# myshell-ai/OpenVoice

Measured on NVIDIA H100. Metric: audio_seconds_per_second, higher is better.
Workload: dtype f32 (3xFP16 split-precision tensor-core convs with fp32 accumulation, fp32 FFMA elsewhere)

## Files before the change

openvoice_b200/csrc/ovc_lib.cu:

```cuda
#include <cuda_runtime.h>

#include <algorithm>
#include <cmath>
#include <cstdarg>
#include <cstdio>
#include <cstdlib>
#include <cstring>
#include <map>
#include <string>
#include <vector>

#include "../../include/ovc.h"
#include "ovc_convpack.h"
#include "ovc_small.cuh"
#include "ovc_tcconv.cuh"
#include "ovc_tts.cuh"
#include "ovc_refenc.cuh"
#include "ovc_resample.cuh"
#include "ovc_splice.h"
#include "ovc_variants.h"

namespace ovc {

static thread_local std::string g_err;
// ... 98 lines not shown
  int n_vocab = 0, n_speakers = 0, H = 0, C = 0, Fc = 0, heads = 0, n_layers = 0, window = 0, D = 0;
  size_t emb = 0, emb_g = 0;
  std::vector<TcLayer> qkv, o;
  std::vector<Fp32Dense> ffn1, ffn2;
  std::vector<size_t> relk, relv, ln1g, ln1b, ln2g, ln2b;
  TcLayer proj;
  Fp32Dense dp_c1, dp_c2, sdp_pre, sdp_proj;
  size_t dp_n1g = 0, dp_n1b = 0, dp_n2g = 0, dp_n2b = 0, dp_pw = 0, dp_pb = 0, dp_cw = 0, dp_cb = 0, sdp_cw = 0, sdp_cb = 0,
         ea = 0;
  DdsLayers dds[4];
  size_t cf_pre_w[4] = {0}, cf_pre_b[4] = {0}, cf_pw[4] = {0}, cf_pb[4] = {0};
};

struct DebugBuf {
  float* d = nullptr;
  int64_t shape[4] = {0, 0, 0, 0};
  size_t floats = 0;
};

}

using namespace ovc;

struct ovc_ctx {
  ovc_hparams hp{};
  int device = 0;
  int sm_count = 0;
  std::map<std::string, HostTensor> sd;
  bool finalized = false;

  float* d_w = nullptr;
  size_t w_floats = 0;
  std::vector<float> h_w;

  ConvLayer enc_pre, enc_pre16, enc_proj;
  WNLayers enc_wn;
  ConvLayer flow_pre[4], flow_post[4];
  WNLayers flow_wn[4];
  ConvLayer dec_pre, dec_ups[4];
  ConvLayer rb_c1[12][3], rb_c2[12][3];
  TcLayer tc_c1[12][3], tc_c2[12][3], tc_ups[4], tc_pre;
  float* d_tcw = nullptr;
  std::vector<float> h_tcw;
  int precision = 0;
  bool tts_simple = false;
  bool use_graph = true;
  int use_pdl = 2;
  bool use_branches = true;
  int par_frames = 512;
  bool use_pair = true;
  bool use_pair_occ = true;
  bool use_staged_epi = true;
  bool pair_occ2_ok[TCN_N_OCC2] = {};
  cudaStream_t br_stream[2] = {nullptr, nullptr};
  cudaEvent_t br_ev[4] = {nullptr, nullptr, nullptr, nullptr};
  size_t post_w_off = 0;
  size_t cond_w_off = 0, cond_b_off = 0;
  int* d_cond_wrow = nullptr;
  int* d_cond_sel = nullptr;
  int cond_rows_out = 0;
  int cond_off_enc = 0, cond_off_fsrc = 0, cond_off_ftgt = 0, cond_off_dec = 0;
  int cond_off_enc_tc = 0, cond_off_fsrc_tc = 0, cond_off_ftgt_tc = 0;
  int* d_cond_cols[2][3] = {};
  int cond_pf_cols[2][3] = {};
  int cond_pf_off[2][3][4] = {};

  float2* d_tw = nullptr;
  float* d_win = nullptr;

  bool has_refenc = false;
  size_t re_conv_w[6] = {0}, re_conv_b[6] = {0}, re_wih = 0, re_whh = 0, re_bih = 0, re_bhh = 0, re_pw = 0, re_pb = 0,
         re_lng = 0, re_lnb = 0;
  int re_gru_in = 0;
  float* d_re = nullptr;
  size_t re_floats = 0;
  float* d_res = nullptr;
  size_t res_floats = 0;

  std::map<std::pair<int64_t, int64_t>, double*> rs_banks;
  bool rs_smem_opt_in = false;
  std::vector<RsRingPlan> rs_plans;
  RsRingPlan* d_rs_plans = nullptr;
  int rs_ring_tile = 256;
  size_t rs_ring_smem = 0;

  float* d_ws = nullptr;
  size_t ws_floats = 0;

  TtsLayers tts;
  float* d_tts = nullptr;
  size_t tts_floats = 0;
  int tts_B = 0, tts_T = 0;
  bool tts_gtok = false;

  bool prof = false;
  std::vector<cudaEvent_t> ev;
  size_t ev_used = 0;
  double prof_ms = 0, prof_flops = 0, prof_bytes = 0;
  int64_t prof_launches = 0;
  std::vector<double> ev_flops, ev_bytes;
  std::vector<int> ev_variant, ev_family, ev_tag;

  bool debug = false;
  std::map<std::string, DebugBuf> taps;

  int launches = 0;
// ... 348 lines not shown
      auto col = [&](int i) { return cols.empty() ? i : cols[i]; };
      for (int i = 0; i < n; ++i)
        if (sel[col(i)] != sel[col(i / COND_ROWS * COND_ROWS)]) return false;
      return true;
    };
    bool ok = uniform({}, (int)sel.size());
    for (auto& oc : pf_cols)
      for (auto& cols : oc) ok = ok && uniform(cols, (int)cols.size());
    if (!ok) return fail(OVC_ERR_INVALID, "conditioning sections are not aligned to %d rows", COND_ROWS);
  }
  c->has_refenc = false;
  if (find(c, "ref_enc.proj.weight")) {
    static const int filt[7] = {1, 32, 32, 64, 64, 128, 128};
    for (int i = 0; i < 6; ++i) {
      const std::string q = "ref_enc.convs." + std::to_string(i);
      HostTensor w;
      const HostTensor* b;
      TRY(conv_weight(c, q, {filt[i + 1], filt[i], 3, 3}, &w));
      TRY(tensor(c, q + ".bias", {filt[i + 1]}, &b));
      c->re_conv_w[i] = append(c->h_w, w.data);
      c->re_conv_b[i] = append(c->h_w, b->data);
    }
    int w6 = S;
    for (int i = 0; i < 6; ++i) w6 = (w6 - 1) / 2 + 1;
    c->re_gru_in = 128 * w6;
    const struct { const char* key; std::vector<int64_t> shape; size_t* off; } re[8] = {
        {"ref_enc.gru.weight_ih_l0", {384, c->re_gru_in}, &c->re_wih}, {"ref_enc.gru.weight_hh_l0", {384, 128}, &c->re_whh},
        {"ref_enc.gru.bias_ih_l0", {384}, &c->re_bih},                 {"ref_enc.gru.bias_hh_l0", {384}, &c->re_bhh},
        {"ref_enc.proj.weight", {G, 128}, &c->re_pw},                  {"ref_enc.proj.bias", {G}, &c->re_pb},
        {"ref_enc.layernorm.weight", {S}, &c->re_lng},                 {"ref_enc.layernorm.bias", {S}, &c->re_lnb}};
    for (const auto& e : re) {
      const HostTensor* t;
      TRY(tensor(c, e.key, e.shape, &t));
      *e.off = append(c->h_w, t->data);
    }
    c->has_refenc = true;
  }
  c->tts = TtsLayers();
  if (find(c, "enc_p.emb.weight")) TRY(pack_tts(c));
  ON_DEVICE(c);
  if (c->d_w) { cudaFree(c->d_w); c->d_w = nullptr; }
  c->w_floats = c->h_w.size();
  CK(cudaMalloc(&c->d_w, c->w_floats * sizeof(float)));
  CK(cudaMemcpy(c->d_w, c->h_w.data(), c->w_floats * sizeof(float), cudaMemcpyHostToDevice));
  if (c->d_tcw) { cudaFree(c->d_tcw); c->d_tcw = nullptr; }
  CK(cudaMalloc(&c->d_tcw, c->h_tcw.size() * sizeof(float)));
  CK(cudaMemcpy(c->d_tcw, c->h_tcw.data(), c->h_tcw.size() * sizeof(float), cudaMemcpyHostToDevice));
  c->h_tcw.clear();
  c->h_tcw.shrink_to_fit();
  for (int TN : {128, 64, 32})
    for (bool staged : {false, true}) {
      const TcKernel k = tc_conv_kernel(TN, staged), p = tc_pair_kernel(TN, TcPairOcc(), staged);
      CK(cudaFuncSetAttribute(k.fn, cudaFuncAttributeMaxDynamicSharedMemorySize, (int)k.smem));
      CK(cudaFuncSetAttribute(p.fn, cudaFuncAttributeMaxDynamicSharedMemorySize, (int)p.smem));
    }
  for (int i = 0; i < TCN_N_OCC2; ++i) {
    const TcKernel k = tc_pair_kernel(kTcPairOcc2[i].C, kTcPairOcc2[i].o);
    CK(cudaFuncSetAttribute(k.fn, cudaFuncAttributeMaxDynamicSharedMemorySize, (int)k.smem));
    int blocks = 0;
    CK(cudaOccupancyMaxActiveBlocksPerMultiprocessor(&blocks, k.fn, k.threads, k.smem));
    c->pair_occ2_ok[i] = blocks >= 2;
    if (blocks < 2)
      fprintf(stderr, "ovc: the C = %d conv-pair kernel with %d operand buffer(s) fits %d CTA(s) per SM, not 2; its pairs run "
              "one CTA per SM\n", kTcPairOcc2[i].C, kTcPairOcc2[i].o.nabuf, blocks);
  }
  if (c->d_cond_wrow) cudaFree(c->d_cond_wrow);
  if (c->d_cond_sel) cudaFree(c->d_cond_sel);
  CK(cudaMalloc(&c->d_cond_wrow, wrow.size() * sizeof(int)));
  CK(cudaMalloc(&c->d_cond_sel, sel.size() * sizeof(int)));
  CK(cudaMemcpy(c->d_cond_wrow, wrow.data(), wrow.size() * sizeof(int), cudaMemcpyHostToDevice));
  CK(cudaMemcpy(c->d_cond_sel, sel.data(), sel.size() * sizeof(int), cudaMemcpyHostToDevice));
  for (int o = 0; o < 2; ++o)
    for (int m = 0; m < 3; ++m) {
      if (c->d_cond_cols[o][m]) cudaFree(c->d_cond_cols[o][m]);
      c->d_cond_cols[o][m] = nullptr;
      if (pf_cols[o][m].empty()) continue;
      CK(cudaMalloc(&c->d_cond_cols[o][m], pf_cols[o][m].size() * sizeof(int)));
      CK(cudaMemcpy(c->d_cond_cols[o][m], pf_cols[o][m].data(), pf_cols[o][m].size() * sizeof(int), cudaMemcpyHostToDevice));
    }
  if (!c->d_tw) {
    std::vector<float2> tw(STFT_N);
    std::vector<float> win(STFT_N);
    const double PI = 3.14159265358979323846;
    for (int m = 0; m < STFT_N; ++m) {
      tw[m] = make_float2((float)std::cos(2.0 * PI * m / STFT_N), (float)(-std::sin(2.0 * PI * m / STFT_N)));
      win[m] = (float)(0.5 - 0.5 * std::cos(2.0 * PI * m / STFT_N));
    }
    CK(cudaMalloc(&c->d_tw, STFT_N * sizeof(float2)));
    CK(cudaMalloc(&c->d_win, STFT_N * sizeof(float)));
    CK(cudaMemcpy(c->d_tw, tw.data(), STFT_N * sizeof(float2), cudaMemcpyHostToDevice));
    CK(cudaMemcpy(c->d_win, win.data(), STFT_N * sizeof(float), cudaMemcpyHostToDevice));
  }
  c->h_w.clear();
  c->h_w.shrink_to_fit();
  c->sd.clear();
  for (int v = 0; v < V_COUNT; ++v) CK(kPrepare[v]());
  c->finalized = true;
  return OVC_OK;
}

struct WsLayout {
  int P;
  size_t cond, cond_pf, g_pf, x, skip, acts, z, dpre, bufA, bufB, bufC, bufD, bufE, bufF, spec, frames, win_g, win_len, total;
  size_t brB[2], brC[2];
  bool branches;
};
static WsLayout ws_layout(const ovc_ctx* c, int B, int Tmax, int pf_cols = 0, bool g_frames = false) {
  WsLayout L;
  L.P = (int)round_up((size_t)Tmax, 4);
  size_t o = 0;
  auto take = [&](size_t n) { size_t r = o; o = round_up(o + n, 64); return r; };
  L.cond = take((size_t)B * c->cond_rows_out);
  L.cond_pf = pf_cols ? take((size_t)B * Tmax * pf_cols) : 0;
  L.g_pf = g_frames ? take((size_t)B * c->hp.gin_channels * Tmax) : 0;
  L.x = take((size_t)B * 192 * L.P);
  L.skip = take((size_t)B * 192 * L.P);
  L.acts = take((size_t)B * 192 * L.P);
// ... 148 lines not shown
  return cudaLaunchKernelEx(&cfg, kernel, std::forward<Args>(args)...);
}

static int launch_tc(Run& r, const TcLayer& T, const float* x, float* y, const float* res, int t_len, int mul, float slope,
                     float scale, int accumulate, int family, const TcExtra& ex = TcExtra()) {
  TcConvArgs a{};
  const int y_ld = ex.y_ld ? ex.y_ld : T.Ntot;
  a.x = x; a.x_bs = (long long)T.Cin * r.P * mul;
  a.w = reinterpret_cast<const uint16_t*>(r.c->d_tcw + T.w_off);
  a.bias = ex.bias ? ex.bias : r.c->d_tcw + T.b_off; a.bias_bs = ex.bias_bs; a.bias_ts = ex.bias_ts;
  a.y = y; a.y_bs = (long long)y_ld * r.P * mul; a.y_ld = y_ld;
  a.r = res;
  a.s = ex.s; a.s_bs = a.y_bs;
  a.epi = ex.epi; a.split = ex.split; a.first = ex.first;
  a.lens = ex.use_lens_frames ? r.lens : r.glens; a.tmax = r.Tmax; a.mul = mul;
  a.lens_x = ex.lens_x; a.has_lens_x = ex.has_lens_x ? 1 : 0;
  a.Cin = T.Cin; a.Ntot = T.Ntot; a.K = T.K; a.DIL = T.DIL;
  a.slope = slope; a.scale = scale; a.accumulate = accumulate;
  a.passes = r.c->precision == 2 ? 1 : 3;
  if (T.TN == 0) return fail(OVC_ERR_INVALID, "conv %d -> %d (k %d, dilation %d) does not fit the tensor-core kernels", T.Cin, T.Ntot, T.K, T.DIL);
  if (!(slope >= 0.f && slope <= 1.f)) return fail(OVC_ERR_INVALID, "leaky_relu slope %g outside [0, 1]", (double)slope);
  TRY(prof_begin(r));
  const TcGrid g = tc_grid(t_len, r.B, T.Ntot, T.TN, r.c->sm_count, ex.grid_div);
  const int n_tt = g.n_tt, total = g.total;
  dim3 pg((unsigned)g.grid_x, g.ncol, 1);
  const bool pdl = r.c->use_pdl == 1 || (r.c->use_pdl == 2 && ex.epi != 0);
  const TcKernel k = tc_conv_kernel(T.TN, r.c->use_staged_epi && tc_stage_pays(T.K, a.passes));
  CK(launch_ex(k.fn, pg, k.threads, k.smem, r.st, pdl, a, n_tt, total));
  CK(cudaGetLastError());
  r.c->launches++;
  const double units = (double)r.B * t_len;
  const int eff_k = family == 2 ? 2 : T.K;
  TRY(prof_end(r, T.TN == 128 ? V_TC128 : T.TN == 64 ? V_TC64 : V_TC32, family == 1 ? 1 : 0, 2.0 * T.Cin * T.Ntot * eff_k * units,
               4.0 * (T.Cin + T.Ntot * (1 + (res ? 1 : 0) + (accumulate ? 1 : 0))) * units, (T.Cin << 16) | (T.K << 8) | T.DIL));
  return OVC_OK;
}

static int launch_pair(Run& r, const TcLayer& T1, const TcLayer& T2, const float* x, float* y, int t_len, int mul, float slope,
                       float scale, int accumulate) {
  TcConvArgs a{};
  const int C = T1.TN;
  a.x = x; a.x_bs = (long long)C * r.P * mul;
  a.w = reinterpret_cast<const uint16_t*>(r.c->d_tcw + T1.w_off);
  a.w2 = reinterpret_cast<const uint16_t*>(r.c->d_tcw + T2.w_off);
  a.bias = r.c->d_tcw + T1.b_off; a.bias2 = r.c->d_tcw + T2.b_off;
  a.y = y; a.y_bs = a.x_bs; a.y_ld = C;
  a.lens = r.glens; a.tmax = r.Tmax; a.mul = mul;
  a.Cin = C; a.Ntot = C; a.K = T1.K; a.DIL = T1.DIL;
  a.slope = slope; a.scale = scale; a.accumulate = accumulate;
  a.passes = r.c->precision == 2 ? 1 : 3;
  TcPairOcc o = r.c->use_pair_occ ? tc_pair_occ(T1, T2) : TcPairOcc();
  for (int i = 0; i < TCN_N_OCC2; ++i)
    if (o.occ == 2 && kTcPairOcc2[i].C == C && kTcPairOcc2[i].o.nabuf == o.nabuf && !r.c->pair_occ2_ok[i]) o = TcPairOcc();
  const TcKernel k = tc_pair_kernel(C, o, r.c->use_staged_epi && tc_stage_pays(T1.K, a.passes));
  if (!k.fn) return fail(OVC_ERR_INVALID, "no conv-pair kernel for C = %d at %d CTA(s) per SM, %d operand buffer(s)", C, o.occ, o.nabuf);
  const TcGrid g = tc_pair_grid(t_len, r.B, T1.K, r.c->sm_count, o.occ);
  const int n_tt = g.n_tt, total = g.total;
  TRY(prof_begin(r));
  dim3 pg((unsigned)g.grid_x, 1, 1);
  CK(launch_ex(k.fn, pg, k.threads, k.smem, r.st, false, a, n_tt, total));
  CK(cudaGetLastError());
  r.c->launches++;
  const double units = (double)r.B * t_len;
  TRY(prof_end(r, C == 128 ? V_TCPAIR128 : C == 64 ? V_TCPAIR64 : V_TCPAIR32, 1, 2.0 * 2.0 * C * C * T1.K * units, 4.0 * C * (2 + (accumulate ? 1 : 0)) * units,
               (C << 16) | (T1.K << 8) | T1.DIL));
  return OVC_OK;
}

static int launch_transpose(Run& r, const float* src, float* dst, int rows, int cols) {
  dim3 grid((cols + 31) / 32, (rows + 31) / 32, r.B);
  TRY(prof_begin(r));
  transpose_kernel<<<grid, 256, 0, r.st>>>(src, dst, rows, cols, (long long)rows * cols);
  CK(cudaGetLastError());
  r.c->launches++;
  TRY(prof_end(r, V_TRANSPOSE, 0, 0.0, 8.0 * rows * cols * r.B));
  return OVC_OK;
}

struct CondRef {
  const float* p; long long bs, ts;
  CondRef at(int col) const { return {p + col, bs, ts}; }
};

static int run_wn(Run& r, const WNLayers& wn, float* x, float* skip, float* acts, const CondRef& cond) {
  const int P = r.P, T = r.Tmax;
  const long long bs = 192LL * P;
  const int n = (int)wn.in.size();
  for (int i = 0; i < n; ++i) {
    ConvArgs a{};
    a.x = x; a.x_bs = bs; a.x_pitch = P;
    a.bias = cond.p + (size_t)i * 384; a.bias_bs = cond.bs; a.bias_ts = cond.ts;
    a.y = acts; a.y_bs = bs; a.y_pitch = P;
    a.lens_in = r.lens; a.lens_out = r.lens; a.mul_in = 1; a.mul_out = 1;
    a.slope = 1.f;
    TRY(launch(r, wn.in[i], a, T));
    ConvArgs b{};
    b.x = acts; b.x_bs = bs; b.x_pitch = P;
    b.bias = r.c->d_w + wn.rs[i].b_off; b.bias_bs = 0;
    b.y = x; b.y_bs = bs; b.y_pitch = P;
    b.s = skip; b.s_bs = bs; b.s_pitch = P;
    b.lens_in = r.lens; b.lens_out = r.lens; b.mul_in = 1; b.mul_out = 1;
    b.slope = 1.f;
    b.split = (i < n - 1) ? 192 : 0;
    b.flags = (i == 0) ? F_FIRST : 0;
    TRY(launch(r, wn.rs[i], b, T));
  }
  return OVC_OK;
}
// ... 1376 lines not shown
```

openvoice_b200/csrc/ovc_tcconv.cuh:

```cuda
#pragma once
#include "ovc_conv.cuh"
#include "ovc_tc.cuh"
#include "ovc_tcpack.h"

namespace ovc {

struct TcConvArgs {
  const float* x; long long x_bs;
  const uint16_t* w;
  const float* bias; long long bias_bs;
  float* y; long long y_bs; int y_ld;
  const float* r;
  float* s; long long s_bs;
  int epi;
  int split; int first;
  const long long* lens; int tmax; int mul;
  const long long* lens_x; int has_lens_x;
  int Cin; int Ntot; int K; int DIL;
  float slope; float scale; int accumulate;
  int passes;
  const uint16_t* w2; const float* bias2;
  long long bias_ts;
};

// ... 77 lines not shown
      const bool add = to_x || !a.first;
      float* dst = (to_x ? yb + col : sb + (col - a.split)) + csub;
#pragma unroll
      for (int g = 0; g < 4; ++g) {
        float2 oa = make_float2(v[4 * g], v[4 * g + 1]), ob = make_float2(v[4 * g + 2], v[4 * g + 3]);
        if (add) {
          const float2 qa = oka ? *reinterpret_cast<const float2*>(dst + (size_t)ta * a.y_ld + 8 * g) : make_float2(0.f, 0.f);
          const float2 qb = okb ? *reinterpret_cast<const float2*>(dst + (size_t)tb * a.y_ld + 8 * g) : make_float2(0.f, 0.f);
          oa = make_float2(qa.x + oa.x, qa.y + oa.y);
          ob = make_float2(qb.x + ob.x, qb.y + ob.y);
        }
        if (oka) *reinterpret_cast<float2*>(dst + (size_t)ta * a.y_ld + 8 * g) = oa;
        if (okb) *reinterpret_cast<float2*>(dst + (size_t)tb * a.y_ld + 8 * g) = ob;
      }
    }
  }
}

template <int TN, class V>
__device__ __forceinline__ void tc_epilogue_v(const TcConvArgs& a, V v_at, int b, int t0, int n0, int lim, int row_a) {
  if (a.bias_ts) tc_epilogue_body<TN, true>(a, v_at, b, t0, n0, lim, row_a);
  else tc_epilogue_body<TN, false>(a, v_at, b, t0, n0, lim, row_a);
}

template <int TN>
__device__ __forceinline__ void tc_epilogue(const TcConvArgs& a, const float (&d)[TN], int b, int t0, int n0, int lim, int row_a) {
  const bool two = a.passes == 3;
  tc_epilogue_v<TN>(a, [&](int j) { return tc_result<TN>(d, two, j); }, b, t0, n0, lim, row_a);
}
__device__ __forceinline__ TcConvArgs tc_pair_epilogue_args(const TcConvArgs& a, int TN) {
  TcConvArgs e = a;
  e.y_ld = TN; e.r = a.x; e.bias = a.bias2; e.bias_bs = 0; e.bias_ts = 0; e.epi = 0;
  return e;
}

template <int TN>
__device__ __forceinline__ void tc_mma_step(float (&d)[TN], uint64_t a_hi, uint64_t a_lo, uint64_t b, bool three, bool first) {
  float (&lo)[TN / 2] = *reinterpret_cast<float(*)[TN / 2]>(&d[TN / 2]);
  float (&hi)[TN / 2] = *reinterpret_cast<float(*)[TN / 2]>(&d[0]);
  tc::Wgmma<TN>::mma(hi, a_hi, b, first ? 0 : 1);
  if (three) {
    tc::Wgmma<TN>::mma(lo, a_hi, b + TN, first ? 0 : 1);
    tc::Wgmma<TN>::mma(lo, a_lo, b, 1);
  }
}

constexpr int TCN_THREADS = 384;
constexpr int TCN_NCT = 96;

template <int TN, bool PAIR, int OCC = 1, int NAB = 2, bool STAGED = false>
struct TcnCfg {
  static_assert(!PAIR || TN == 32 || TN == 64 || TN == 128, "conv pairs: C = 32, 64 or 128");
  static_assert(OCC == 1 || (PAIR && TN <= 64), "two CTAs per SM: C = 32 / 64 pairs");
  static_assert(!STAGED || (TN == 128 && OCC == 1), "staged epilogue: TN = 128, one CTA per SM");
  static constexpr int THREADS = STAGED ? TCN_THREADS + 128 : TCN_THREADS;
  static constexpr int KCH = 32, NKC = KCH / 8;
  static constexpr int ROWS = 194;
  static constexpr int ROWS2 = TCN_ROWS2;
  static constexpr int NABUF = NAB;
  static constexpr int RING = PAIR ? tc_pair_ring(TN, OCC, NAB) : tc_ring_slots(TN, PAIR);
  static constexpr int SLOT_BYTES = 2 * 2 * TN * 16;
  static constexpr int A_BUF_BYTES = 2 * NKC * ROWS * 16;
  static constexpr int A2_BYTES = PAIR ? 2 * (TN / 8) * ROWS2 * 16 : 0;
  static constexpr int STAGE_BYTES = STAGED ? (TN / 2) * 256 * 4 : 0;
  static_assert(!STAGED || !PAIR || STAGE_BYTES <= A2_BYTES, "a pair's staging tile lies in its conv-2 operand");
  static constexpr int SBUF_BYTES = STAGED && !PAIR ? STAGE_BYTES : 0;
  static constexpr size_t SMEM_BYTES = 1024 + NABUF * A_BUF_BYTES + A2_BYTES + RING * SLOT_BYTES + SBUF_BYTES;
  static_assert(!PAIR || SMEM_BYTES == tc_pair_smem(TN, NABUF, RING), "tc_pair_smem");
  static_assert(SMEM_BYTES <= (OCC == 1 ? 232448 : TCN_SMEM_OCC2), "shared memory budget");
  static_assert((2 * NABUF + 2 * RING + 2) * 8 <= 1024, "barrier area");
  static constexpr int PROD_REGS = OCC == 1 && !STAGED ? 56 : 32, MMA_REGS = STAGED ? 184 : OCC == 1 ? 224 : 104;
  static constexpr int STORE_REGS = 112;
  static_assert(128 * PROD_REGS + 256 * MMA_REGS + (STAGED ? 128 * STORE_REGS : 0) <= 65536 / OCC, "register budget");
};

template <int TN, bool PAIR, int OCC = 1, int NAB = 2, bool STAGED = false>
__global__ void __launch_bounds__(TcnCfg<TN, PAIR, OCC, NAB, STAGED>::THREADS, OCC) tcconv_kernel(const TcConvArgs a, int n_tt, int total) {
  using Cfg = TcnCfg<TN, PAIR, OCC, NAB, STAGED>;
  constexpr int ROWS = Cfg::ROWS, ROWS2 = Cfg::ROWS2, NABUF = Cfg::NABUF, RING = Cfg::RING, NKC = Cfg::NKC;
  extern __shared__ __align__(128) unsigned char smem_raw[];
  uint64_t* bars = reinterpret_cast<uint64_t*>(smem_raw);
  uint64_t *a_full = bars, *a_empty = bars + NABUF, *b_full = a_empty + NABUF, *b_empty = b_full + RING;
  uint64_t *s_full = b_empty + RING, *s_empty = s_full + 1;
  unsigned char* abuf = smem_raw + 1024;
  unsigned char* a2buf = abuf + NABUF * Cfg::A_BUF_BYTES;
  unsigned char* bring = a2buf + Cfg::A2_BYTES;
  float* stage = reinterpret_cast<float*>(PAIR ? a2buf : bring + RING * Cfg::SLOT_BYTES);

  const int tid = threadIdx.x, lane = tid & 31;
  const int warp = __shfl_sync(0xffffffffu, tid >> 5, 0);
  const int H1 = (a.K - 1) / 2 * a.DIL;
  const int H2 = PAIR ? (a.K - 1) / 2 : 0;
  const int R = 128 - 2 * H2;
  const int rows8 = (128 + 2 * H1 + 7) & ~7;
  const int nq = a.Cin / Cfg::KCH;
  const int n_slots = (a.Cin / 16) * a.K;
  const int n_w = PAIR ? 2 * n_slots : n_slots;
  const bool resident = n_w <= RING;
  if (H1 > TCN_HMAX || (PAIR && 128 + 2 * H2 > ROWS2)) __trap();
  constexpr uint32_t BYTES = Cfg::SLOT_BYTES;

  if (tid == 0) {
    for (int i = 0; i < NABUF; ++i) { mbar_init(&a_full[i], TCN_NCT); mbar_init(&a_empty[i], 2); }
    for (int i = 0; i < RING; ++i) { mbar_init(&b_full[i], 1); mbar_init(&b_empty[i], 2); }
    if (STAGED) { mbar_init(s_full, 256); mbar_init(s_empty, 128); }
    fence_mbar_init();
  }
  if (PAIR) {
    for (int i = tid; i < Cfg::A2_BYTES / 16; i += Cfg::THREADS) reinterpret_cast<uint4*>(a2buf)[i] = make_uint4(0u, 0u, 0u, 0u);
    asm volatile("fence.proxy.async.shared::cta;" ::: "memory");
  }
  __syncthreads();
  pdl_launch_dependents();
  if (warp != 0) pdl_wait();

#define TCN_FOR_TILES                                                                                   \
  for (int tile = blockIdx.x; tile < total; tile += gridDim.x) {                                        \
    const int b = tile / n_tt, t0 = (tile % n_tt) * R;                                                  \
    const int lim = (a.lens ? (int)min((long long)a.tmax, a.lens[b]) : a.tmax) * a.mul;                 \
    const int lim_x = a.has_lens_x ? (int)min((long long)a.tmax, a.lens_x[b]) * a.mul : lim;            \
    (void)lim_x;                                                                                        \
    if (t0 >= lim) continue;

  if (warp < 4) {
    tc::regs_dealloc<Cfg::PROD_REGS>();
    if (warp == 0) {
      if (lane == 0) {
        const unsigned char* wt = reinterpret_cast<const unsigned char*>(a.w) + (size_t)blockIdx.y * n_slots * BYTES;
        if (resident) {
          for (int it = 0; it < n_w; ++it) {
            const unsigned char* src = it < n_slots ? wt + (size_t)it * BYTES
                                                    : reinterpret_cast<const unsigned char*>(a.w2) + (size_t)(it - n_slots) * BYTES;
            mbar_expect_tx(&b_full[it], BYTES);
            tma_bulk_g2s(bring + it * BYTES, src, BYTES, &b_full[it]);
          }
          for (int it = 0; it < n_w; ++it) mbar_wait(&b_full[it], 0u);
        } else {
          int slot = 0;
          uint32_t phase = 1;
          TCN_FOR_TILES
            (void)b;
            for (int it = 0; it < n_w; ++it) {
              const unsigned char* src = it < n_slots ? wt + (size_t)it * BYTES
                                                      : reinterpret_cast<const unsigned char*>(a.w2) + (size_t)(it - n_slots) * BYTES;
              mbar_wait(&b_empty[slot], phase);
              mbar_expect_tx(&b_full[slot], BYTES);
              tma_bulk_g2s(bring + slot * BYTES, src, BYTES, &b_full[slot]);
              if (++slot == RING) { slot = 0; phase ^= 1; }
            }
          }
        }
      }
    } else {
      const int pt = tid - 32;
      const int items = rows8 * NKC;
      int buf = 0;
      uint32_t ephase = 1;
      TCN_FOR_TILES
        const float* xb = a.x + (size_t)b * a.x_bs;
        const int r0 = t0 - H2 - H1;
        for (int q = 0; q < nq; ++q) {
          mbar_wait(&a_empty[buf], ephase);
          unsigned char* ah = abuf + buf * Cfg::A_BUF_BYTES;
          unsigned char* al = ah + NKC * ROWS * 16;
          constexpr int PB = 2;
          for (int i0 = pt; i0 < items; i0 += TCN_NCT * PB) {
            float4 v0[PB], v1[PB];
#pragma unroll
            for (int u = 0; u < PB; ++u) {
              const int i = i0 + TCN_NCT * u;
              const int row = i >> 2, kc = i & 3;
              const int t = r0 + row;
              v0[u] = make_float4(0.f, 0.f, 0.f, 0.f);
              v1[u] = v0[u];
              if (i < items && t >= 0 && t < lim_x) {
                const float4* src = reinterpret_cast<const float4*>(xb + (size_t)t * a.Cin + q * Cfg::KCH + kc * 8);
                v0[u] = src[0];
                v1[u] = src[1];
              }
            }
#pragma unroll
            for (int u = 0; u < PB; ++u) {
              const int i = i0 + TCN_NCT * u;
              if (i >= items) break;
              const int row = i >> 2, kc = i & 3;
              uint4 hi, lo;
              tc::split_f16x8(v0[u], v1[u], a.slope, hi, lo);
              *reinterpret_cast<uint4*>(ah + (kc * ROWS + row) * 16) = hi;
              *reinterpret_cast<uint4*>(al + (kc * ROWS + row) * 16) = lo;
            }
          }
          asm volatile("fence.proxy.async.shared::cta;" ::: "memory");
          mbar_arrive(&a_full[buf]);
          if (++buf == NABUF) { buf = 0; ephase ^= 1; }
        }
      }
    }
  } else if (STAGED && warp >= 12) {
    tc::regs_dealloc<Cfg::STORE_REGS>();
    const int st = tid & 127;
    uint32_t phase = 0;
    TCN_FOR_TILES
      if (PAIR) named_bar_arrive(1, 384);
      mbar_wait(s_full, phase);
      phase ^= 1;
#pragma unroll 1
      for (int h = 0; h < 2; ++h) {
        const float* sv = stage + h * 128 + st;
        const auto v_at = [&](int j) { return sv[j * 256]; };
        const int row_a = 64 * h + 16 * (warp & 3) + (lane >> 2);
        if constexpr (PAIR) tc_epilogue_v<TN>(tc_pair_epilogue_args(a, TN), v_at, b, t0, 0, min(lim, t0 + R), row_a);
        else tc_epilogue_v<TN>(a, v_at, b, t0, blockIdx.y * TN, lim, row_a);
      }
      if (!PAIR) mbar_arrive(s_empty);
    }
  } else {
    tc::regs_alloc<Cfg::MMA_REGS>();
    const int wg = (warp >> 2) - 1;
    const bool leader = (tid & 127) == 0;
    const int row_a = 64 * wg + 16 * (warp & 3) + (lane >> 2);
    constexpr uint32_t LBO_A = ROWS * 16, LBO_A2 = ROWS2 * 16, LBO_B = 2 * TN * 16, SBO = 128;
    constexpr uint32_t A_LO16 = (NKC * ROWS * 16) >> 4, A2_LO16 = ((TN / 8) * ROWS2 * 16) >> 4, SLOT16 = BYTES >> 4;
    const uint64_t a_proto = tc::make_desc(0, LBO_A, SBO), b_proto = tc::make_desc(0, LBO_B, SBO);
    const uint64_t b_ring = b_proto + (tc::smem_addr(bring) >> 4);
    const bool three = a.passes == 3;
    float d[TN];
#pragma unroll
    for (int i = 0; i < TN; ++i) d[i] = 0.f;
    const auto stage_tile = [&]() {
#pragma unroll
      for (int j = 0; j < TN / 2; ++j) stage[j * 256 + tid - 128] = tc_result<TN>(d, three, j);
      mbar_arrive(s_full);
    };
    uint32_t sphase = 1;
    (void)sphase;
    if (resident)
      for (int it = 0; it < n_w; ++it) mbar_wait(&b_full[it], 0u);
    int slot = 0, buf = 0;
    uint32_t bphase = 0, aphase = 0;
    TCN_FOR_TILES
      (void)lim_x;
      bool first = true;
      if (resident) slot = 0;
      for (int q = 0; q < nq; ++q) {
        mbar_wait(&a_full[buf], aphase);
        tc::fence_regs(d);
        tc::wgmma_fence();
        int prev = -1;
        for (int j = 0; j < 2; ++j) {
          uint64_t a_cur = a_proto + ((tc::smem_addr(abuf + buf * Cfg::A_BUF_BYTES) + 64 * wg * 16 + 2 * j * LBO_A) >> 4);
          for (int tap = 0; tap < a.K; ++tap) {
            if (!resident) mbar_wait(&b_full[slot], bphase);
            tc_mma_step<TN>(d, a_cur, a_cur + A_LO16, b_ring + (uint32_t)slot * SLOT16, three, first);
            tc::wgmma_commit();
            if (!resident) {
              tc::wgmma_wait<1>();
              if (leader && prev >= 0) mbar_arrive(&b_empty[prev]);
              prev = slot;
            }
            first = false;
            a_cur += a.DIL;
            if (++slot == RING) { slot = 0; bphase ^= 1; }
          }
        }
        tc::wgmma_wait<0>();
        tc::fence_regs(d);
        if (leader) {
          if (prev >= 0) mbar_arrive(&b_empty[prev]);
          mbar_arrive(&a_empty[buf]);
        }
        if (++buf == NABUF) { buf = 0; aphase ^= 1; }
      }
      if constexpr (!PAIR) {
        if constexpr (STAGED) {
          mbar_wait(s_empty, sphase);
          sphase ^= 1;
          stage_tile();
        } else {
          tc_epilogue<TN>(a, d, b, t0, blockIdx.y * TN, lim, row_a);
        }
      } else {
        named_bar_sync(1, STAGED ? 384 : 256);
        unsigned char* a2h = a2buf;
        unsigned char* a2l = a2buf + (TN / 8) * ROWS2 * 16;
        const int ta = t0 - H2 + row_a, tb = ta + 8;
        const bool oka = ta >= 0 && ta < lim, okb = tb >= 0 && tb < lim;
        const int csub = (lane & 3) * 2;
#pragma unroll
        for (int g = 0; g < TN / 8; ++g) {
          const float2 bq = __ldg(reinterpret_cast<const float2*>(a.bias + 8 * g + csub));
          float x[4];
#pragma unroll
          for (int i = 0; i < 4; ++i) x[i] = (three ? fmaf(d[TN / 2 + 4 * g + i], tc::kLoInv, d[4 * g + i]) : d[4 * g + i]) + ((i & 1) ? bq.y : bq.x);
          x[0] = oka ? fmaxf(x[0], x[0] * a.slope) : 0.f;
          x[1] = oka ? fmaxf(x[1], x[1] * a.slope) : 0.f;
          x[2] = okb ? fmaxf(x[2], x[2] * a.slope) : 0.f;
          x[3] = okb ? fmaxf(x[3], x[3] * a.slope) : 0.f;
          const __half2 ha = __floats2half2_rn(x[0], x[1]), hb = __floats2half2_rn(x[2], x[3]);
          const float2 fa = __half22float2(ha), fb = __half22float2(hb);
          const __half2 la = __floats2half2_rn((x[0] - fa.x) * tc::kLoScale, (x[1] - fa.y) * tc::kLoScale);
          const __half2 lb = __floats2half2_rn((x[2] - fb.x) * tc::kLoScale, (x[3] - fb.y) * tc::kLoScale);
          const int oa = (g * ROWS2 + row_a) * 16 + (lane & 3) * 4, ob = oa + 8 * 16;
          *reinterpret_cast<__half2*>(a2h + oa) = ha;
          *reinterpret_cast<__half2*>(a2h + ob) = hb;
          *reinterpret_cast<__half2*>(a2l + oa) = la;
          *reinterpret_cast<__half2*>(a2l + ob) = lb;
        }
        asm volatile("fence.proxy.async.shared::cta;" ::: "memory");
        named_bar_sync(2, 256);
        const uint64_t a2_proto = tc::make_desc(0, LBO_A2, SBO);
        tc::fence_regs(d);
        tc::wgmma_fence();
        bool first2 = true;
        int prev = -1;
        for (int kk = 0; kk < TN / 16; ++kk) {
          uint64_t a_cur = a2_proto + ((tc::smem_addr(a2buf) + 64 * wg * 16 + 2 * kk * LBO_A2) >> 4);
          for (int tap = 0; tap < a.K; ++tap) {
            if (resident) {
              tc_mma_step<TN>(d, a_cur, a_cur + A2_LO16, b_ring + (uint32_t)(n_slots + kk * a.K + tap) * SLOT16, three, first2);
            } else {
              mbar_wait(&b_full[slot], bphase);
              tc_mma_step<TN>(d, a_cur, a_cur + A2_LO16, b_ring + (uint32_t)slot * SLOT16, three, first2);
              tc::wgmma_commit();
              tc::wgmma_wait<1>();
              if (leader && prev >= 0) mbar_arrive(&b_empty[prev]);
              prev = slot;
              if (++slot == RING) { slot = 0; bphase ^= 1; }
            }
            first2 = false;
            a_cur += 1;
          }
        }
        tc::wgmma_commit();
        tc::wgmma_wait<0>();
        tc::fence_regs(d);
        if (leader && prev >= 0) mbar_arrive(&b_empty[prev]);
        if constexpr (STAGED) {
          named_bar_sync(3, 256);
          stage_tile();
        } else {
          tc_epilogue<TN>(tc_pair_epilogue_args(a, TN), d, b, t0, 0, min(lim, t0 + R), row_a);
        }
      }
    }
  }
#undef TCN_FOR_TILES
}

struct TcKernel {
  void (*fn)(TcConvArgs, int, int) = nullptr;
  size_t smem = 0;
  int threads = 0;
};
using TcPairKernel = TcKernel;
template <int TN, bool PAIR, int OCC = 1, int NAB = 2, bool STAGED = false>
inline TcKernel tc_kernel() {
  using Cfg = TcnCfg<TN, PAIR, OCC, NAB, STAGED>;
  return {tcconv_kernel<TN, PAIR, OCC, NAB, STAGED>, Cfg::SMEM_BYTES, Cfg::THREADS};
}
inline bool tc_stage_pays(int K, int passes) { return passes * K >= 15; }
inline TcKernel tc_conv_kernel(int TN, bool staged) {
  if (TN == 128) return staged ? tc_kernel<128, false, 1, 2, true>() : tc_kernel<128, false>();
  if (TN == 64) return tc_kernel<64, false>();
  if (TN == 32) return tc_kernel<32, false>();
  return {};
}
inline TcKernel tc_pair_kernel(int C, TcPairOcc o, bool staged = false) {
  if (o.occ == 1 && o.nabuf == 2) {
    if (C == 128) return staged ? tc_kernel<128, true, 1, 2, true>() : tc_kernel<128, true>();
    if (C == 64) return tc_kernel<64, true>();
    if (C == 32) return tc_kernel<32, true>();
  } else if (o.occ == 2) {
    if (C == 32 && o.nabuf == 2) return tc_kernel<32, true, 2, 2>();
    if (C == 32 && o.nabuf == 1) return tc_kernel<32, true, 2, 1>();
    if (C == 64 && o.nabuf == 1) return tc_kernel<64, true, 2, 1>();
  }
  return {};
}
constexpr int TCN_N_OCC2 = 3;
constexpr struct { int C; TcPairOcc o; } kTcPairOcc2[TCN_N_OCC2] = {{32, {2, 2}}, {32, {2, 1}}, {64, {2, 1}}};

template <int C>
__global__ void __launch_bounds__(256) conv_post_cl_kernel(const float* __restrict__ x, long long x_bs,
                                                           const float* __restrict__ w, float* __restrict__ y,
                                                           long long y_bs, int y_len, const long long* lens, int tmax,
                                                           int mul) {
  constexpr int TB = 256, ROWS = TB + 6, LD = ROWS + 3;
  __shared__ float ws[7][C];
  __shared__ float xs[C][LD];
  for (int i = threadIdx.x; i < C * 7; i += blockDim.x) ws[i % 7][i / 7] = w[i];
  const int b = blockIdx.y;
  const int lim = (lens ? (int)min((long long)tmax, lens[b]) : tmax) * mul;
  const int t0 = blockIdx.x * TB;
  const float* xb = x + (size_t)b * x_bs;
  for (int idx = threadIdx.x; idx < ROWS * (C / 4); idx += blockDim.x) {
    const int row = idx / (C / 4), q = idx % (C / 4);
    const int tt = t0 - 3 + row;
    float4 v = make_float4(0.f, 0.f, 0.f, 0.f);
    if (tt >= 0 && tt < lim) v = *reinterpret_cast<const float4*>(xb + (size_t)tt * C + 4 * q);
    xs[4 * q + 0][row] = v.x > 0.f ? v.x : 0.01f * v.x;
    xs[4 * q + 1][row] = v.y > 0.f ? v.y : 0.01f * v.y;
    xs[4 * q + 2][row] = v.z > 0.f ? v.z : 0.01f * v.z;
    xs[4 * q + 3][row] = v.w > 0.f ? v.w : 0.01f * v.w;
  }
  __syncthreads();
  const int t = t0 + threadIdx.x;
  if (t >= y_len) return;
  float acc = 0.f;
  if (t < lim) {
#pragma unroll
    for (int k = 0; k < 7; ++k)
#pragma unroll 8
      for (int ci = 0; ci < C; ++ci) acc = fmaf(ws[k][ci], xs[ci][threadIdx.x + k], acc);
    acc = tanhf(acc);
  }
  y[(size_t)b * y_bs + t] = acc;
}

__global__ void __launch_bounds__(256) transpose_kernel(const float* __restrict__ src, float* __restrict__ dst, int rows,
                                                        int cols, long long bs) {
  __shared__ float tile[32][33];
  const float* s = src + (size_t)blockIdx.z * bs;
  float* d = dst + (size_t)blockIdx.z * bs;
  const int c0 = blockIdx.x * 32, r0 = blockIdx.y * 32;
// ... 14 lines not shown
```

openvoice_b200/csrc/ovc_tcpack.h:

```cpp
#pragma once
#include <cuda_fp16.h>
#include <stddef.h>
#include <stdint.h>

#include <algorithm>

namespace ovc {

constexpr int TCN_HMAX = 25;
constexpr int TCN_ROWS2 = 146;

constexpr int tc_ring_slots(int TN, bool pair) {
  return pair ? (TN == 32 ? 44 : TN == 64 ? 24 : 12) : (TN == 32 ? 22 : 12);
}

struct TcGeom {
  int Cin = 0, Ntot = 0, K = 0, DIL = 1, TN = 0;
};

inline int tc_tile_n(int Ntot, int Cin, int K, int DIL) {
  if (Ntot <= 0 || Cin <= 0 || K <= 0 || DIL <= 0) return 0;
  if (Ntot % 32 || Cin % 32 || (K - 1) / 2 * DIL > TCN_HMAX) return 0;
  return Ntot % 128 == 0 ? 128 : (Ntot % 64 == 0 ? 64 : 32);
}
// ... 25 lines not shown
          for (int n = 0; n < TN; ++n)
            for (int e = 0; e < 8; ++e) {
              uint16_t hi, lo;
              tc_split(wfun(nt * TN + n, k16 * 16 + kc * 8 + e, tap), hi, lo);
              sl[((kc * 2 + 0) * TN + n) * 8 + e] = hi;
              sl[((kc * 2 + 1) * TN + n) * 8 + e] = lo;
            }
      }
}

template <class RAW>
inline float tc_ups_weight(RAW raw, int s, int kk, int cout, int row, int ci, int tap) {
  const int pad = (kk - s) / 2;
  const int ph = row / cout, co = row % cout;
  const int kidx = s * (1 - tap) + ph + pad;
  return (kidx >= 0 && kidx < kk) ? raw(ci, co, kidx) : 0.f;
}

inline bool tc_pair_fits(const TcGeom& T1, const TcGeom& T2) {
  if (!(T1.TN == 32 || T1.TN == 64)) return false;
  const int ring = tc_ring_slots(T1.TN, true);
  return T1.Ntot == T1.TN && T1.Cin == T1.TN && T2.Ntot == T1.TN && T2.Cin == T1.TN && T2.TN == T1.TN && T2.K == T1.K &&
         T2.DIL == 1 && (T1.K - 1) / 2 * T1.DIL <= TCN_HMAX && 2 * (T1.Cin / 16) * T1.K <= ring && T1.K <= 5;
}

inline bool tc_pair_fuses(const TcGeom& T1, const TcGeom& T2) {
  if (!(T1.TN == 32 || T1.TN == 64 || T1.TN == 128)) return false;
  return T1.Ntot == T1.TN && T1.Cin == T1.TN && T2.Ntot == T1.TN && T2.Cin == T1.TN && T2.TN == T1.TN && T2.K == T1.K &&
         T2.DIL == 1 && (T1.K - 1) / 2 * T1.DIL <= TCN_HMAX && 128 + 2 * ((T2.K - 1) / 2) <= TCN_ROWS2;
}

struct TcGrid {
  int n_tt = 0, total = 0, grid_x = 0, ncol = 0;
};
inline TcGrid tc_grid(int t_len, int B, int Ntot, int TN, int sm_count, int grid_div) {
  TcGrid g;
  g.n_tt = (t_len + 127) / 128;
  g.total = g.n_tt * B;
  g.ncol = Ntot / TN;
  const int per_col = std::max(1, sm_count / g.ncol / std::max(1, grid_div));
  g.grid_x = std::min(g.total, per_col);
  return g;
}
inline TcGrid tc_pair_grid(int t_len, int B, int K, int sm_count, int occ = 1) {
  TcGrid g;
  const int R = 128 - (K - 1);
  g.n_tt = (t_len + R - 1) / R;
  g.total = g.n_tt * B;
  g.ncol = 1;
  g.grid_x = std::min(g.total, occ * sm_count);
  return g;
}

constexpr size_t tc_pair_smem(int TN, int nabuf, int ring) {
  return 1024 + (size_t)nabuf * 2 * 4 * 194 * 16 + (size_t)2 * (TN / 8) * TCN_ROWS2 * 16 + (size_t)ring * 2 * 2 * TN * 16;
}
constexpr size_t TCN_SMEM_OCC2 = (233472 - 2 * 1024) / 2;
constexpr int tc_pair_ring(int TN, int occ, int nabuf) {
  return occ == 1 ? tc_ring_slots(TN, true) : (int)((TCN_SMEM_OCC2 - tc_pair_smem(TN, nabuf, 0)) / (2 * 2 * TN * 16));
}

struct TcPairOcc {
  int occ = 1, nabuf = 2;
};
inline TcPairOcc tc_pair_occ(const TcGeom& T1, const TcGeom& T2) {
  TcPairOcc o;
  if (!tc_pair_fuses(T1, T2)) return o;
  const int n_w = 2 * (T1.Cin / 16) * T1.K;
  if (T1.TN == 32 && n_w <= tc_pair_ring(32, 2, 2)) o = {2, 2};
  else if (T1.TN == 32 && n_w <= tc_pair_ring(32, 2, 1)) o = {2, 1};
  else if (T1.TN == 64 && n_w > tc_pair_ring(64, 1, 2)) o = {2, 1};
  return o;
}

}
```

Baseline: 2413.

## Add double-buffered staged epilogue for C=32 conv-pair kernels

```diff
diff --git a/openvoice_b200/csrc/ovc_lib.cu b/openvoice_b200/csrc/ovc_lib.cu
--- a/openvoice_b200/csrc/ovc_lib.cu
+++ b/openvoice_b200/csrc/ovc_lib.cu
@@ -174,6 +174,7 @@
   bool use_pair_occ = true;
   bool use_staged_epi = true;
   bool pair_occ2_ok[TCN_N_OCC2] = {};
+  bool pair32_staged_ok = false;
   cudaStream_t br_stream[2] = {nullptr, nullptr};
   cudaEvent_t br_ev[4] = {nullptr, nullptr, nullptr, nullptr};
   size_t post_w_off = 0;
@@ -628,7 +629,7 @@
     for (bool staged : {false, true}) {
       const TcKernel k = tc_conv_kernel(TN, staged), p = tc_pair_kernel(TN, TcPairOcc(), staged);
       CK(cudaFuncSetAttribute(k.fn, cudaFuncAttributeMaxDynamicSharedMemorySize, (int)k.smem));
-      CK(cudaFuncSetAttribute(p.fn, cudaFuncAttributeMaxDynamicSharedMemorySize, (int)p.smem));
+      if (p.fn) CK(cudaFuncSetAttribute(p.fn, cudaFuncAttributeMaxDynamicSharedMemorySize, (int)p.smem));
     }
   for (int i = 0; i < TCN_N_OCC2; ++i) {
     const TcKernel k = tc_pair_kernel(kTcPairOcc2[i].C, kTcPairOcc2[i].o);
@@ -639,6 +640,14 @@
     if (blocks < 2)
       fprintf(stderr, "ovc: the C = %d conv-pair kernel with %d operand buffer(s) fits %d CTA(s) per SM, not 2; its pairs run "
               "one CTA per SM\n", kTcPairOcc2[i].C, kTcPairOcc2[i].o.nabuf, blocks);
+  }
+  {
+    const TcKernel k = tc_pair_kernel(32, TcPairOcc(), true);
+    int blocks = 0;
+    CK(cudaOccupancyMaxActiveBlocksPerMultiprocessor(&blocks, k.fn, k.threads, k.smem));
+    c->pair32_staged_ok = blocks == 1;
+    if (blocks != 1)
+      fprintf(stderr, "ovc: the staged C = 32 conv-pair kernel fits %d CTA(s) per SM, not 1; its pairs are not staged\n", blocks);
   }
   if (c->d_cond_wrow) cudaFree(c->d_cond_wrow);
   if (c->d_cond_sel) cudaFree(c->d_cond_sel);
@@ -893,8 +902,10 @@
   TcPairOcc o = r.c->use_pair_occ ? tc_pair_occ(T1, T2) : TcPairOcc();
   for (int i = 0; i < TCN_N_OCC2; ++i)
     if (o.occ == 2 && kTcPairOcc2[i].C == C && kTcPairOcc2[i].o.nabuf == o.nabuf && !r.c->pair_occ2_ok[i]) o = TcPairOcc();
-  const TcKernel k = tc_pair_kernel(C, o, r.c->use_staged_epi && tc_stage_pays(T1.K, a.passes));
-  if (!k.fn) return fail(OVC_ERR_INVALID, "no conv-pair kernel for C = %d at %d CTA(s) per SM, %d operand buffer(s)", C, o.occ, o.nabuf);
+  const bool staged = r.c->use_staged_epi && tc_pair_stage(T1, T2, a.passes) && (C != 32 || r.c->pair32_staged_ok);
+  const TcKernel k = tc_pair_kernel(C, o, staged);
+  if (!k.fn) return fail(OVC_ERR_INVALID, "no conv-pair kernel for C = %d at %d CTA(s) per SM, %d operand buffer(s)%s", C, o.occ,
+                         o.nabuf, staged ? ", staged" : "");
   const TcGrid g = tc_pair_grid(t_len, r.B, T1.K, r.c->sm_count, o.occ);
   const int n_tt = g.n_tt, total = g.total;
   TRY(prof_begin(r));
diff --git a/openvoice_b200/csrc/ovc_tcconv.cuh b/openvoice_b200/csrc/ovc_tcconv.cuh
--- a/openvoice_b200/csrc/ovc_tcconv.cuh
+++ b/openvoice_b200/csrc/ovc_tcconv.cuh
@@ -153,23 +153,27 @@
 struct TcnCfg {
   static_assert(!PAIR || TN == 32 || TN == 64 || TN == 128, "conv pairs: C = 32, 64 or 128");
   static_assert(OCC == 1 || (PAIR && TN <= 64), "two CTAs per SM: C = 32 / 64 pairs");
-  static_assert(!STAGED || (TN == 128 && OCC == 1), "staged epilogue: TN = 128, one CTA per SM");
+  static_assert(!STAGED || (OCC == 1 && (TN == 128 || (PAIR && NAB == 2))),
+                "staged epilogue: one CTA per SM; TN = 128, or a C = 32 / 64 pair with two operand buffers");
   static constexpr int THREADS = STAGED ? TCN_THREADS + 128 : TCN_THREADS;
   static constexpr int KCH = 32, NKC = KCH / 8;
   static constexpr int ROWS = 194;
   static constexpr int ROWS2 = TCN_ROWS2;
   static constexpr int NABUF = NAB;
-  static constexpr int RING = PAIR ? tc_pair_ring(TN, OCC, NAB) : tc_ring_slots(TN, PAIR);
+  static constexpr int NSB = STAGED ? (PAIR && TN < 128 ? 2 : 1) : 0;
+  static constexpr int NST = PAIR && TN < 128 ? NSB : 0;
+  static constexpr int RING = PAIR ? tc_pair_ring(TN, OCC, NAB, NST) : tc_ring_slots(TN, PAIR);
   static constexpr int SLOT_BYTES = 2 * 2 * TN * 16;
   static constexpr int A_BUF_BYTES = 2 * NKC * ROWS * 16;
   static constexpr int A2_BYTES = PAIR ? 2 * (TN / 8) * ROWS2 * 16 : 0;
   static constexpr int STAGE_BYTES = STAGED ? (TN / 2) * 256 * 4 : 0;
-  static_assert(!STAGED || !PAIR || STAGE_BYTES <= A2_BYTES, "a pair's staging tile lies in its conv-2 operand");
-  static constexpr int SBUF_BYTES = STAGED && !PAIR ? STAGE_BYTES : 0;
+  static constexpr bool OVERLAY = STAGED && PAIR && TN == 128;
+  static_assert(!OVERLAY || STAGE_BYTES <= A2_BYTES, "a pair's staging tile lies in its conv-2 operand");
+  static constexpr int SBUF_BYTES = STAGED && !OVERLAY ? NSB * STAGE_BYTES : 0;
   static constexpr size_t SMEM_BYTES = 1024 + NABUF * A_BUF_BYTES + A2_BYTES + RING * SLOT_BYTES + SBUF_BYTES;
-  static_assert(!PAIR || SMEM_BYTES == tc_pair_smem(TN, NABUF, RING), "tc_pair_smem");
-  static_assert(SMEM_BYTES <= (OCC == 1 ? 232448 : TCN_SMEM_OCC2), "shared memory budget");
-  static_assert((2 * NABUF + 2 * RING + 2) * 8 <= 1024, "barrier area");
+  static_assert(!PAIR || SMEM_BYTES == tc_pair_smem(TN, NABUF, RING, NST), "tc_pair_smem");
+  static_assert(SMEM_BYTES <= (OCC == 1 ? TCN_SMEM_OCC1 : TCN_SMEM_OCC2), "shared memory budget");
+  static_assert((2 * NABUF + 2 * RING + 2 * (NSB ? NSB : 1)) * 8 <= 1024, "barrier area");
   static constexpr int PROD_REGS = OCC == 1 && !STAGED ? 56 : 32, MMA_REGS = STAGED ? 184 : OCC == 1 ? 224 : 104;
   static constexpr int STORE_REGS = 112;
   static_assert(128 * PROD_REGS + 256 * MMA_REGS + (STAGED ? 128 * STORE_REGS : 0) <= 65536 / OCC, "register budget");
@@ -178,15 +182,16 @@
 template <int TN, bool PAIR, int OCC = 1, int NAB = 2, bool STAGED = false>
 __global__ void __launch_bounds__(TcnCfg<TN, PAIR, OCC, NAB, STAGED>::THREADS, OCC) tcconv_kernel(const TcConvArgs a, int n_tt, int total) {
   using Cfg = TcnCfg<TN, PAIR, OCC, NAB, STAGED>;
-  constexpr int ROWS = Cfg::ROWS, ROWS2 = Cfg::ROWS2, NABUF = Cfg::NABUF, RING = Cfg::RING, NKC = Cfg::NKC;
+  constexpr int ROWS = Cfg::ROWS, ROWS2 = Cfg::ROWS2, NABUF = Cfg::NABUF, RING = Cfg::RING, NKC = Cfg::NKC, NSB = Cfg::NSB;
+  constexpr bool OVERLAY = Cfg::OVERLAY;
   extern __shared__ __align__(128) unsigned char smem_raw[];
   uint64_t* bars = reinterpret_cast<uint64_t*>(smem_raw);
   uint64_t *a_full = bars, *a_empty = bars + NABUF, *b_full = a_empty + NABUF, *b_empty = b_full + RING;
-  uint64_t *s_full = b_empty + RING, *s_empty = s_full + 1;
+  uint64_t *s_full = b_empty + RING, *s_empty = s_full + (NSB ? NSB : 1);
   unsigned char* abuf = smem_raw + 1024;
   unsigned char* a2buf = abuf + NABUF * Cfg::A_BUF_BYTES;
   unsigned char* bring = a2buf + Cfg::A2_BYTES;
-  float* stage = reinterpret_cast<float*>(PAIR ? a2buf : bring + RING * Cfg::SLOT_BYTES);
+  float* stage = reinterpret_cast<float*>(OVERLAY ? a2buf : bring + RING * Cfg::SLOT_BYTES);
 
   const int tid = threadIdx.x, lane = tid & 31;
   const int warp = __shfl_sync(0xffffffffu, tid >> 5, 0);
@@ -204,7 +209,7 @@
   if (tid == 0) {
     for (int i = 0; i < NABUF; ++i) { mbar_init(&a_full[i], TCN_NCT); mbar_init(&a_empty[i], 2); }
     for (int i = 0; i < RING; ++i) { mbar_init(&b_full[i], 1); mbar_init(&b_empty[i], 2); }
-    if (STAGED) { mbar_init(s_full, 256); mbar_init(s_empty, 128); }
+    for (int i = 0; i < NSB; ++i) { mbar_init(&s_full[i], 256); mbar_init(&s_empty[i], 128); }
     fence_mbar_init();
   }
   if (PAIR) {
@@ -300,20 +305,22 @@
   } else if (STAGED && warp >= 12) {
     tc::regs_dealloc<Cfg::STORE_REGS>();
     const int st = tid & 127;
+    int sb = 0;
     uint32_t phase = 0;
     TCN_FOR_TILES
-      if (PAIR) named_bar_arrive(1, 384);
-      mbar_wait(s_full, phase);
-      phase ^= 1;
+      if (OVERLAY) named_bar_arrive(1, 384);
+      mbar_wait(&s_full[sb], phase);
+      const int cur = sb;
+      if (++sb == NSB) { sb = 0; phase ^= 1; }
 #pragma unroll 1
       for (int h = 0; h < 2; ++h) {
-        const float* sv = stage + h * 128 + st;
+        const float* sv = stage + cur * (Cfg::STAGE_BYTES / 4) + h * 128 + st;
         const auto v_at = [&](int j) { return sv[j * 256]; };
         const int row_a = 64 * h + 16 * (warp & 3) + (lane >> 2);
         if constexpr (PAIR) tc_epilogue_v<TN>(tc_pair_epilogue_args(a, TN), v_at, b, t0, 0, min(lim, t0 + R), row_a);
         else tc_epilogue_v<TN>(a, v_at, b, t0, blockIdx.y * TN, lim, row_a);
       }
-      if (!PAIR) mbar_arrive(s_empty);
+      if (!OVERLAY) mbar_arrive(&s_empty[cur]);
     }
   } else {
     tc::regs_alloc<Cfg::MMA_REGS>();
@@ -328,13 +335,16 @@
     float d[TN];
 #pragma unroll
     for (int i = 0; i < TN; ++i) d[i] = 0.f;
+    int sb = 0;
+    uint32_t sphase = 1;
+    (void)sb; (void)sphase;
     const auto stage_tile = [&]() {
-#pragma unroll
-      for (int j = 0; j < TN / 2; ++j) stage[j * 256 + tid - 128] = tc_result<TN>(d, three, j);
-      mbar_arrive(s_full);
+      float* sv = stage + sb * (Cfg::STAGE_BYTES / 4);
+#pragma unroll
+      for (int j = 0; j < TN / 2; ++j) sv[j * 256 + tid - 128] = tc_result<TN>(d, three, j);
+      mbar_arrive(&s_full[sb]);
+      if (++sb == NSB) { sb = 0; sphase ^= 1; }
     };
-    uint32_t sphase = 1;
-    (void)sphase;
     if (resident)
       for (int it = 0; it < n_w; ++it) mbar_wait(&b_full[it], 0u);
     int slot = 0, buf = 0;
@@ -374,14 +384,13 @@
       }
       if constexpr (!PAIR) {
         if constexpr (STAGED) {
-          mbar_wait(s_empty, sphase);
-          sphase ^= 1;
+          mbar_wait(&s_empty[sb], sphase);
           stage_tile();
         } else {
           tc_epilogue<TN>(a, d, b, t0, blockIdx.y * TN, lim, row_a);
         }
       } else {
-        named_bar_sync(1, STAGED ? 384 : 256);
+        named_bar_sync(1, OVERLAY ? 384 : 256);
         unsigned char* a2h = a2buf;
         unsigned char* a2l = a2buf + (TN / 8) * ROWS2 * 16;
         const int ta = t0 - H2 + row_a, tb = ta + 8;
@@ -436,8 +445,11 @@
         tc::wgmma_wait<0>();
         tc::fence_regs(d);
         if (leader && prev >= 0) mbar_arrive(&b_empty[prev]);
-        if constexpr (STAGED) {
+        if constexpr (OVERLAY) {
           named_bar_sync(3, 256);
+          stage_tile();
+        } else if constexpr (STAGED) {
+          mbar_wait(&s_empty[sb], sphase);
           stage_tile();
         } else {
           tc_epilogue<TN>(tc_pair_epilogue_args(a, TN), d, b, t0, 0, min(lim, t0 + R), row_a);
@@ -460,6 +472,10 @@
   return {tcconv_kernel<TN, PAIR, OCC, NAB, STAGED>, Cfg::SMEM_BYTES, Cfg::THREADS};
 }
 inline bool tc_stage_pays(int K, int passes) { return passes * K >= 15; }
+inline bool tc_pair_stage(const TcGeom& T1, const TcGeom& T2, int passes) {
+  if (T1.TN == 128) return tc_stage_pays(T1.K, passes);
+  return T1.TN == 32 && tc_pair_fuses(T1, T2) && tc_pair_occ(T1, T2).occ == 1;
+}
 inline TcKernel tc_conv_kernel(int TN, bool staged) {
   if (TN == 128) return staged ? tc_kernel<128, false, 1, 2, true>() : tc_kernel<128, false>();
   if (TN == 64) return tc_kernel<64, false>();
@@ -469,8 +485,8 @@
 inline TcKernel tc_pair_kernel(int C, TcPairOcc o, bool staged = false) {
   if (o.occ == 1 && o.nabuf == 2) {
     if (C == 128) return staged ? tc_kernel<128, true, 1, 2, true>() : tc_kernel<128, true>();
-    if (C == 64) return tc_kernel<64, true>();
-    if (C == 32) return tc_kernel<32, true>();
+    if (C == 64) return staged ? TcKernel() : tc_kernel<64, true>();
+    if (C == 32) return staged ? tc_kernel<32, true, 1, 2, true>() : tc_kernel<32, true>();
   } else if (o.occ == 2) {
     if (C == 32 && o.nabuf == 2) return tc_kernel<32, true, 2, 2>();
     if (C == 32 && o.nabuf == 1) return tc_kernel<32, true, 2, 1>();
diff --git a/openvoice_b200/csrc/ovc_tcpack.h b/openvoice_b200/csrc/ovc_tcpack.h
--- a/openvoice_b200/csrc/ovc_tcpack.h
+++ b/openvoice_b200/csrc/ovc_tcpack.h
@@ -101,12 +101,15 @@
   return g;
 }
 
-constexpr size_t tc_pair_smem(int TN, int nabuf, int ring) {
-  return 1024 + (size_t)nabuf * 2 * 4 * 194 * 16 + (size_t)2 * (TN / 8) * TCN_ROWS2 * 16 + (size_t)ring * 2 * 2 * TN * 16;
+constexpr size_t tc_pair_smem(int TN, int nabuf, int ring, int nst = 0) {
+  return 1024 + (size_t)nabuf * 2 * 4 * 194 * 16 + (size_t)2 * (TN / 8) * TCN_ROWS2 * 16 + (size_t)ring * 2 * 2 * TN * 16 +
+         (size_t)nst * (TN / 2) * 256 * 4;
 }
 constexpr size_t TCN_SMEM_OCC2 = (233472 - 2 * 1024) / 2;
-constexpr int tc_pair_ring(int TN, int occ, int nabuf) {
-  return occ == 1 ? tc_ring_slots(TN, true) : (int)((TCN_SMEM_OCC2 - tc_pair_smem(TN, nabuf, 0)) / (2 * 2 * TN * 16));
+constexpr size_t TCN_SMEM_OCC1 = 232448;
+constexpr int tc_pair_ring(int TN, int occ, int nabuf, int nst = 0) {
+  return occ == 2 ? (int)((TCN_SMEM_OCC2 - tc_pair_smem(TN, nabuf, 0)) / (2 * 2 * TN * 16))
+                  : std::min(tc_ring_slots(TN, true), (int)((TCN_SMEM_OCC1 - tc_pair_smem(TN, nabuf, 0, nst)) / (2 * 2 * TN * 16)));
 }
 
 struct TcPairOcc {
```

New measurement: 2431 (median of 6 runs). About the same (+0.8%).
